# hackmad/pbrt-v3-rs

Measured on AMD Instinct MI355X. Metric: Mrays/s, higher is better.
Workload: dtype f32

## Files before the change

### pbrt-v3-rs_amd/csrc/api.hip

```cpp
#include "host_math.h"
#include "scene_host.h"
#include "traverse.h"
#include "texture.h"
#include <algorithm>
#include <cstdio>
#include <cstdlib>
#include <mutex>

static std::string g_last_error;
static std::mutex g_err_mu;

namespace phost {

int set_err(PbrtHipScene* s, int code, const std::string& msg) {
    if (s) s->err = msg;
    else { std::lock_guard<std::mutex> g(g_err_mu); g_last_error = msg; }
    return code;
}
int hip_fail(PbrtHipScene* s, hipError_t e, const char* what) {
    std::string m = std::string(what) + ": " + hipGetErrorString(e);
    (void)hipGetLastError();
    return set_err(s, e == hipErrorOutOfMemory ? PBRT_HIP_ERR_OOM : PBRT_HIP_ERR_DEVICE, m);
}
int ensure_buf(PbrtHipScene* s, DevBuf& b, size_t bytes) {
// ... 1351 lines not shown
            std::string e;
            const phost::ForestSpec spec = layout.spec(isc);
            const int brc = split_method == 1 ? phost::build_hlbvh_device(in, max_prims_in_node, s->stream, s->bvh, e, &spec, &trees)
                                              : phost::build_sah_device(in, max_prims_in_node, s->stream, s->bvh, e, &s->tree_dev_nodes, &s->tree_dev_tris, &spec, &trees);
            if (brc == -1) return set_err(s, PBRT_HIP_ERR_DEVICE, "build_accel_device: " + e);
            if (brc != 0) return fail(brc);
            if (s->tree_dev_tris) s->tree_dev_n_tris = layout.items.size();
        } else {
            const int brc = phost::build_forest_host(in, isc, layout, split_method, max_prims_in_node, s->bvh, trees);
            if (brc != 0) return fail(brc);
        }
        for (size_t k = 0; k < s->instances.size(); k++) {
            const PbrtHipScene::InstanceHost& ih = s->instances[k];
            const phost::ForestTreeOut& b = trees[layout.inst_tree[k]];
            InstRec r{};
            std::memcpy(r.w2i, ih.w2i, 64); std::memcpy(r.i2w, ih.i2w, 64);
            for (int a = 0; a < 3; a++) { r.lo[a] = b.lo[a]; r.hi[a] = b.hi[a]; }
            r.root_ref = b.root_ref; r.flags = b.n_items == 1 ? PH_INST_SINGLE : 0u;
            bool ident = true;
            for (int a = 0; a < 16; a++) if (ih.i2w[a] != ((a % 5 == 0) ? 1.0f : 0.0f)) ident = false;
            if (ident) r.flags |= PH_INST_IDENTITY;
            s->inst_recs.push_back(r);
        }
    }
    s->world_radius = 1.0f; s->world_center[0] = s->world_center[1] = s->world_center[2] = 0.0f;
    if (s->bvh.root_ref != PH_INVALID_REF) {
        const float* lo = s->bvh.root_lo; const float* hi = s->bvh.root_hi;
        float c[3];
        for (int k = 0; k < 3; k++) c[k] = (1.0f - 0.5f) * lo[k] + 0.5f * hi[k];
        bool inside = (c[0] >= lo[0] && c[0] <= hi[0]) && (c[1] >= lo[1] && c[1] <= hi[1]) && (c[2] >= lo[2] && c[2] <= hi[2]);
        float dx = c[0] - hi[0], dy = c[1] - hi[1], dz = c[2] - hi[2];
        s->world_radius = inside ? std::sqrt(dx * dx + dy * dy + dz * dz) : 0.0f;
        for (int k = 0; k < 3; k++) s->world_center[k] = c[k];
    }
    s->built = true; s->uploaded = false;
    return PBRT_HIP_OK;
    });
}

int pbrt_hip_build_accel_device(PbrtHipScene* s, int split_method, int max_prims_in_node) {
    return ph_guard(s, "pbrt_hip_build_accel_device", [&]() -> int {
    if (!s) return PBRT_HIP_ERR_INVALID_ARG;
    if (split_method != 0 && split_method != 1) return set_err(s, PBRT_HIP_ERR_UNSUPPORTED, "build_accel_device: the device builders make the SAH (0) and the HLBVH (1) tree; EqualCounts is built on the host");
    s->build_on_device = true;
    const int rc = pbrt_hip_build_accel(s, split_method, max_prims_in_node);
    s->build_on_device = false;
    return rc;
    });
}

int pbrt_hip_world_bound(const PbrtHipScene* s, float out[6]) {
    return ph_guard(const_cast<PbrtHipScene*>(s), "pbrt_hip_world_bound", [&]() -> int {
    if (!s || !out) return PBRT_HIP_ERR_INVALID_ARG;
    if (!s->built) return PBRT_HIP_ERR_STATE;
    for (int k = 0; k < 3; k++) { out[k] = s->bvh.root_lo[k]; out[3 + k] = s->bvh.root_hi[k]; }
    return PBRT_HIP_OK;
    });
}

int pbrt_hip_accel_stats(const PbrtHipScene* s, uint64_t out[8]) {
    return ph_guard(const_cast<PbrtHipScene*>(s), "pbrt_hip_accel_stats", [&]() -> int {
    if (!s || !out) return PBRT_HIP_ERR_INVALID_ARG;
    if (!s->built) return PBRT_HIP_ERR_STATE;
    out[0] = s->tree_dev_tris ? s->bvh.interior_nodes : s->bvh.nodes.size(); out[1] = s->tree_dev_tris ? s->tree_dev_n_tris : s->bvh.tris.size();
    out[2] = out[0] * sizeof(Node64); out[3] = out[1] * sizeof(TriRec);
    out[4] = s->bvh.leaf_nodes; out[5] = (uint64_t)s->bvh.max_depth; out[6] = s->bvh.max_leaf_prims;
    out[7] = (uint64_t)(s->bvh.build_seconds * 1e6);
    return PBRT_HIP_OK;
    });
}

int pbrt_hip_accel_copy(PbrtHipScene* s, void* out_nodes, uint64_t node_capacity, void* out_leaf_records, uint64_t record_capacity) {
    return ph_guard(s, "pbrt_hip_accel_copy", [&]() -> int {
    if (!s) return PBRT_HIP_ERR_INVALID_ARG;
    if (!s->built) return set_err(s, PBRT_HIP_ERR_STATE, "accel_copy: build_accel first");
    const size_t nn = s->tree_dev_tris ? s->bvh.interior_nodes : s->bvh.nodes.size(), nt = s->tree_dev_tris ? s->tree_dev_n_tris : s->bvh.tris.size();
    if (node_capacity < nn || record_capacity < nt) return set_err(s, PBRT_HIP_ERR_INVALID_ARG, "accel_copy: buffers too small (pbrt_hip_accel_stats gives the sizes)");
    if (s->tree_dev_tris) {
        PH_CHECK(s, hipSetDevice(s->device));
        if (nn && out_nodes) PH_CHECK(s, hipMemcpy(out_nodes, s->tree_dev_nodes, nn * sizeof(Node64), hipMemcpyDeviceToHost));
        if (nt && out_leaf_records) PH_CHECK(s, hipMemcpy(out_leaf_records, s->tree_dev_tris, nt * sizeof(TriRec), hipMemcpyDeviceToHost));
        if (!s->inst_recs.empty()) {
            if (out_nodes) { Node64* nd = static_cast<Node64*>(out_nodes); for (size_t i = 0; i < nn; i++) { if ((nd[i].c0 & PH_LEAF_BIT) && nd[i].c0 < PH_NEED_POP) nd[i].c0 &= ~PH_LEAF_INST_HINT; if ((nd[i].c1 & PH_LEAF_BIT) && nd[i].c1 < PH_NEED_POP) nd[i].c1 &= ~PH_LEAF_INST_HINT; } }
            if (out_leaf_records) { TriRec* tr = static_cast<TriRec*>(out_leaf_records); for (size_t i = 0; i < nt; i++) { tr[i].flags &= ~PH_TRI_NEXT_INST; if (tr[i].flags & PH_TRI_INSTANCE) { const uint32_t prim = tr[i].prim, fl = tr[i].flags; std::memset(&tr[i], 0, sizeof(TriRec)); tr[i].prim = prim; tr[i].flags = fl; } } }
        }
    } else {
        if (nn && out_nodes) std::memcpy(out_nodes, s->bvh.nodes.data(), nn * sizeof(Node64));
        if (nt && out_leaf_records) std::memcpy(out_leaf_records, s->bvh.tris.data(), nt * sizeof(TriRec));
    }
    return PBRT_HIP_OK;
    });
}

static int check_error_flag(PbrtHipScene* s) {
    uint32_t flag = 0;
    PH_CHECK(s, hipMemcpy(&flag, s->d_error.p, 4, hipMemcpyDeviceToHost));
    if (flag) {
        (void)hipMemset(s->d_error.p, 0, 4);
        return set_err(s, PBRT_HIP_ERR_DEVICE, "traversal stack exceeded 64 entries (the reference panics here, bvh/mod.rs:185)");
    }
    return PBRT_HIP_OK;
}

static int batch_common(PbrtHipScene* s, bool anyhit, const void* rays, void* out, uint64_t n, bool device_ptrs, float* kernel_ms) {
    if (!s) return PBRT_HIP_ERR_INVALID_ARG;
    if (n && (!rays || !out)) return set_err(s, PBRT_HIP_ERR_INVALID_ARG, "batch: null buffer");
    if (!s->built) return set_err(s, PBRT_HIP_ERR_STATE, "batch: call pbrt_hip_build_accel first");
    if (n > 0xFFFF0000ull) return set_err(s, PBRT_HIP_ERR_INVALID_ARG, "batch: at most 2^32-65536 rays per call");
    PH_CHECK(s, hipSetDevice(s->device));
    int rc;
    if ((rc = upload_scene(s))) return rc;
    if (n == 0) return PBRT_HIP_OK;
    const size_t out_bytes = anyhit ? (size_t)n : (size_t)n * sizeof(PbrtHipHit);
    const void* d_rays = rays; void* d_out = out;
    if (!device_ptrs) {
        if ((rc = ensure_buf(s, s->d_rays_tmp, (size_t)n * sizeof(PbrtHipRay)))) return rc;
        if ((rc = ensure_buf(s, s->d_out_tmp, out_bytes))) return rc;
        PH_CHECK(s, hipMemcpyAsync(s->d_rays_tmp.p, rays, (size_t)n * sizeof(PbrtHipRay), hipMemcpyHostToDevice, s->stream));
        d_rays = s->d_rays_tmp.p; d_out = s->d_out_tmp.p;
    }
    if ((rc = launch_traverse(s, anyhit, d_rays, d_out, (uint32_t)n, kernel_ms))) return rc;
    if (!device_ptrs) PH_CHECK(s, hipMemcpyAsync(out, d_out, out_bytes, hipMemcpyDeviceToHost, s->stream));
    PH_CHECK(s, hipStreamSynchronize(s->stream));
    return check_error_flag(s);
}

int pbrt_hip_intersect_batch(PbrtHipScene* s, const PbrtHipRay* rays, PbrtHipHit* hits, uint64_t n) { return ph_guard(s, "pbrt_hip_intersect_batch", [&]() -> int { return batch_common(s, false, rays, hits, n, false, nullptr); }); }
int pbrt_hip_occluded_batch(PbrtHipScene* s, const PbrtHipRay* rays, uint8_t* out, uint64_t n) { return ph_guard(s, "pbrt_hip_occluded_batch", [&]() -> int { return batch_common(s, true, rays, out, n, false, nullptr); }); }
int pbrt_hip_intersect_batch_device(PbrtHipScene* s, const void* d_rays, void* d_hits, uint64_t n, float* ms) { return ph_guard(s, "pbrt_hip_intersect_batch_device", [&]() -> int { return batch_common(s, false, d_rays, d_hits, n, true, ms); }); }
int pbrt_hip_occluded_batch_device(PbrtHipScene* s, const void* d_rays, void* d_occ, uint64_t n, float* ms) { return ph_guard(s, "pbrt_hip_occluded_batch_device", [&]() -> int { return batch_common(s, true, d_rays, d_occ, n, true, ms); }); }

int pbrt_hip_set_traversal_counting(PbrtHipScene* s, int on) {
    return ph_guard(s, "pbrt_hip_set_traversal_counting", [&]() -> int {
    if (!s) return PBRT_HIP_ERR_INVALID_ARG;
    PH_CHECK(s, hipSetDevice(s->device));
    int rc;
    if ((rc = ensure_traversal_workspace(s))) return rc;
    PH_CHECK(s, hipMemset(s->d_counts.p, 0, 64 + 36 * 8));
    s->count_traversal = on != 0;
    return PBRT_HIP_OK;
    });
}
int pbrt_hip_get_traversal_counts(PbrtHipScene* s, uint64_t out[8]) {
    return ph_guard(s, "pbrt_hip_get_traversal_counts", [&]() -> int {
    if (!s || !out) return PBRT_HIP_ERR_INVALID_ARG;
    if (!s->d_counts.p) { for (int i = 0; i < 8; i++) out[i] = 0; return PBRT_HIP_OK; }
    PH_CHECK(s, hipSetDevice(s->device));
    PH_CHECK(s, hipStreamSynchronize(s->stream));
    PH_CHECK(s, hipMemcpy(out, s->d_counts.p, 64, hipMemcpyDeviceToHost));
#if PH_PHASE_CLOCK
    {
        unsigned long long ph[36];
        PH_CHECK(s, hipMemcpy(ph, (const char*)s->d_counts.p + 64, sizeof ph, hipMemcpyDeviceToHost));
        static const char* names[10] = {"refill", "node_steps", "instance_entry", "triangle_test", "alpha_test", "instance_exit", "retire", "whole_loop", "stack_pops", "leaf_step_whole"};
        for (int k = 0; k < 10; k++)
            std::fprintf(stderr, "PHASE_CLOCK %-15s cycles %14llu (%5.1f %% of the loop)  executions %12llu  mean active lanes %5.1f\n", names[k], ph[k], ph[7] ? 100.0 * (double)ph[k] / (double)ph[7] : 0.0,
                         ph[12 + k], ph[12 + k] ? (double)ph[24 + k] / (double)ph[12 + k] : 0.0);
    }
    PH_CHECK(s, hipMemset(s->d_counts.p, 0, 64 + 36 * 8));
#else
    PH_CHECK(s, hipMemset(s->d_counts.p, 0, 64 + 36 * 8));
#endif
    return PBRT_HIP_OK;
    });
}

int pbrt_hip_film_to_rgb(const PbrtHipScene* s, const float* xyz, const float* weight, float* out_rgb) {
    return ph_guard(const_cast<PbrtHipScene*>(s), "pbrt_hip_film_to_rgb", [&]() -> int {
    if (!s || !xyz || !weight || !out_rgb) return PBRT_HIP_ERR_INVALID_ARG;
    if (!s->have_film) return PBRT_HIP_ERR_STATE;
    const FilmRec& f = s->film;
    const int w = f.crop[2] - f.crop[0], h = f.crop[3] - f.crop[1];
    const size_t n = (size_t)std::max(w, 0) * (size_t)std::max(h, 0);
    auto to_rgb = [](const float* x, float* r) {
        r[0] = 3.240479f * x[0] - 1.537150f * x[1] - 0.498535f * x[2];
        r[1] = -0.969256f * x[0] + 1.875991f * x[1] + 0.041556f * x[2];
        r[2] = 0.055648f * x[0] - 0.204043f * x[1] + 1.057311f * x[2];
    };
    const float zero[3] = {0, 0, 0};
    float splat_rgb[3];
    to_rgb(zero, splat_rgb);
    for (size_t i = 0; i < n; i++) {
        float rgb[3];
        to_rgb(xyz + 3 * i, rgb);
        for (int c = 0; c < 3; c++) {
            float v = rgb[c];
            if (weight[i] != 0.0f) { float inv = 1.0f / weight[i]; float q = v * inv; v = 0.0f > q ? 0.0f : q; }
            v += 1.0f * splat_rgb[0];
            v *= f.scale;
            out_rgb[3 * i + c] = v;
        }
    }
    return PBRT_HIP_OK;
    });
}

}
```

### pbrt-v3-rs_amd/csrc/traverse.h

```cpp
#pragma once
#include "dmath.h"
#include "scene_types.h"
#include "quadric.h"

constexpr int PH_TRAV_BLOCK = 256;
constexpr int PH_MAX_STACK = 64;
constexpr int PH_BATCH = 64;

namespace ph {

struct alignas(16) RayIn { float ox, oy, oz, t_max, dx, dy, dz, time; };
struct alignas(16) HitOut { float t; uint32_t prim; float b0, b1, b2; uint32_t pad[3]; };

typedef float ph_v4f __attribute__((ext_vector_type(4)));
static __device__ __forceinline__ float4 ph_stream_load(const float4* p) { const ph_v4f v = __builtin_nontemporal_load(reinterpret_cast<const ph_v4f*>(p)); return make_float4(v.x, v.y, v.z, v.w); }
static __device__ __forceinline__ uint32_t ph_stream_load(const uint32_t* p) { return __builtin_nontemporal_load(p); }
static __device__ __forceinline__ void ph_stream_store(float4 v, float4* p) { const ph_v4f w = {v.x, v.y, v.z, v.w}; __builtin_nontemporal_store(w, reinterpret_cast<ph_v4f*>(p)); }
struct TravParams {
    const RayIn* rays;
    void* out;
    uint32_t n;
    const uint32_t* n_ptr;
    uint32_t* counter;
    uint2* spill;
    uint32_t total_threads;
    uint32_t* error_flag;
    uint32_t batch;
    unsigned long long* counts;
    const RayIn* rays2; uint8_t* out2; const uint32_t* n2_ptr;
    const uint32_t* order;
    uint32_t* heads; uint32_t n_heads, head_chunk;
    unsigned long long* phase;
};

struct RayState {
    float ox, oy, oz, t_max;
    float ix, iy, iz;
    uint32_t sgn;
    float sx, sy, sz;
    PH_DEV bool nx() const { return (sgn & 1u) != 0u; }
    PH_DEV bool ny() const { return (sgn & 2u) != 0u; }
    PH_DEV bool nz() const { return (sgn & 4u) != 0u; }
    PH_DEV int kz() const { return (int)((sgn >> 3) & 3u); }
    PH_DEV int kx() const { const int k = kz() + 1; return k == 3 ? 0 : k; }
    PH_DEV int ky() const { const int k = kx() + 1; return k == 3 ? 0 : k; }
};

PH_DEV void ray_setup(RayState& r, const RayIn& in) {
    r.ox = in.ox; r.oy = in.oy; r.oz = in.oz; r.t_max = in.t_max;
    r.ix = 1.0f / in.dx; r.iy = 1.0f / in.dy; r.iz = 1.0f / in.dz;
    f3 d = mk3(in.dx, in.dy, in.dz);
    const int kz = max_dimension(vabs(d));
    r.sgn = (r.ix < 0.0f ? 1u : 0u) | (r.iy < 0.0f ? 2u : 0u) | (r.iz < 0.0f ? 4u : 0u) | ((uint32_t)kz << 3);
    f3 dp = permute(d, r.kx(), r.ky(), kz);
    r.sx = -dp.x / dp.z; r.sy = -dp.y / dp.z; r.sz = 1.0f / dp.z;
}

PH_DEV RayIn xf_ray(const float* c, const RayState& r, f3 rd, float time) {
    const float x = r.ox, y = r.oy, z = r.oz;
    const float ox = (c[0] * x + c[1] * y) + (c[2] * z + c[3]);
    const float oy = (c[4] * x + c[5] * y) + (c[6] * z + c[7]);
    const float oz = (c[8] * x + c[9] * y) + (c[10] * z + c[11]);
    const float ow = (c[12] * x + c[13] * y) + (c[14] * z + c[15]);
    const float xs = pabs(c[0] * x) + pabs(c[1] * y) + pabs(c[2] * z) + pabs(c[3]);
    const float ys = pabs(c[4] * x) + pabs(c[5] * y) + pabs(c[6] * z) + pabs(c[7]);
    const float zs = pabs(c[8] * x) + pabs(c[9] * y) + pabs(c[10] * z) + pabs(c[11]);
    const f3 o_err = kGamma3 * mk3(xs, ys, zs);
    f3 o = (ow == 1.0f) ? mk3(ox, oy, oz) : mk3(ox, oy, oz) / ow;
    const f3 d = mk3(c[0] * rd.x + c[1] * rd.y + c[2] * rd.z, c[4] * rd.x + c[5] * rd.y + c[6] * rd.z, c[8] * rd.x + c[9] * rd.y + c[10] * rd.z);
    const float l2 = length_squared(d);
    float t_max = r.t_max;
    if (l2 > 0.0f) {
        const float dt = ph_div(dot(vabs(d), o_err), l2);
        o = o + d * dt;
        t_max -= dt;
    }
    RayIn out; out.ox = o.x; out.oy = o.y; out.oz = o.z; out.t_max = t_max; out.dx = d.x; out.dy = d.y; out.dz = d.z; out.time = time;
    return out;
}

PH_DEV float vmax3(float a, float b, float c) {
#if defined(__HIP_DEVICE_COMPILE__)
    float r; asm("v_max3_f32 %0, %1, %2, %3" : "=v"(r) : "v"(a), "v"(b), "v"(c)); return r;
#else
    return a > b ? (a > c ? a : c) : (b > c ? b : c);
#endif
}
PH_DEV float vmin3(float a, float b, float c) {
#if defined(__HIP_DEVICE_COMPILE__)
    float r; asm("v_min3_f32 %0, %1, %2, %3" : "=v"(r) : "v"(a), "v"(b), "v"(c)); return r;
#else
    return a < b ? (a < c ? a : c) : (b < c ? b : c);
#endif
}

PH_DEV bool box_test(const RayState& r, float xn, float xf, float yn, float yf, float zn, float zf, float& t_min_out) {
    float t_x_min = (xn - r.ox) * r.ix;
    float t_x_max = (xf - r.ox) * r.ix;
    const float t_y_min = (yn - r.oy) * r.iy;
    float t_y_max = (yf - r.oy) * r.iy;
    t_x_max *= kBoxScale;
    t_y_max *= kBoxScale;
    const float t_z_min = (zn - r.oz) * r.iz;
    const float t_z_max = (zf - r.oz) * r.iz;
    const float t_min = vmax3(t_x_min, t_y_min, t_z_min);
    const float t_max = vmin3(t_x_max, t_y_max, t_z_max);
    t_min_out = t_min;
    return (t_min <= t_max) & (t_max > 0.0f) & ((t_x_min == t_x_min) & (t_x_max == t_x_max));
}

typedef float ph_v2f __attribute__((ext_vector_type(2)));
typedef unsigned long long ph_mask;
PH_DEV ph_mask lanes(bool c) {
#if defined(__HIP_DEVICE_COMPILE__)
    return __ballot(c);
#else
    return c ? 1ull : 0ull;
#endif
}
PH_DEV bool lane_of(ph_mask m) {
#if defined(__HIP_DEVICE_COMPILE__)
    return __builtin_amdgcn_inverse_ballot_w64(m);
#else
    return (m & 1ull) != 0ull;
#endif
}
template <int SEL> PH_DEV ph_v2f pk_sub_bcast(ph_v2f a, ph_v2f p) {
#if defined(__HIP_DEVICE_COMPILE__)
    ph_v2f d;
    if (SEL == 0) asm("v_pk_add_f32 %0, %1, %2 op_sel_hi:[1,0] neg_lo:[0,1] neg_hi:[0,1]" : "=v"(d) : "v"(a), "v"(p));
    else asm("v_pk_add_f32 %0, %1, %2 op_sel:[0,1] op_sel_hi:[1,1] neg_lo:[0,1] neg_hi:[0,1]" : "=v"(d) : "v"(a), "v"(p));
    return d;
#else
    const float o = SEL ? p.y : p.x; return (ph_v2f){a.x - o, a.y - o};
#endif
}
template <int SEL> PH_DEV ph_v2f pk_mul_bcast(ph_v2f a, ph_v2f p) {
#if defined(__HIP_DEVICE_COMPILE__)
    ph_v2f d;
    if (SEL == 0) asm("v_pk_mul_f32 %0, %1, %2 op_sel_hi:[1,0]" : "=v"(d) : "v"(a), "v"(p));
    else asm("v_pk_mul_f32 %0, %1, %2 op_sel:[0,1] op_sel_hi:[1,1]" : "=v"(d) : "v"(a), "v"(p));
    return d;
#else
    const float o = SEL ? p.y : p.x; return (ph_v2f){a.x * o, a.y * o};
#endif
}
PH_DEV void node_boxes(const RayState& r, float4 q0, float4 q1, float4 q2, ph_mask& m0, float& t0, ph_mask& m1, float& t1) {
    const ph_v2f pxy = {r.ox, r.oy}, pzi = {r.oz, r.ix}, pii = {r.iy, r.iz};
    const ph_v2f ax = pk_mul_bcast<1>(pk_sub_bcast<0>((ph_v2f){q0.x, q0.y}, pxy), pzi), ay = pk_mul_bcast<0>(pk_sub_bcast<1>((ph_v2f){q0.z, q0.w}, pxy), pii),
                 az = pk_mul_bcast<1>(pk_sub_bcast<0>((ph_v2f){q1.x, q1.y}, pzi), pii);
    const ph_v2f bx = pk_mul_bcast<1>(pk_sub_bcast<0>((ph_v2f){q1.z, q1.w}, pxy), pzi), by = pk_mul_bcast<0>(pk_sub_bcast<1>((ph_v2f){q2.x, q2.y}, pxy), pii),
                 bz = pk_mul_bcast<1>(pk_sub_bcast<0>((ph_v2f){q2.z, q2.w}, pzi), pii);
    const bool nx = r.nx(), ny = r.ny(), nz = r.nz();
    const ph_v2f scale = {kBoxScale, kBoxScale};
    const ph_v2f a_far = (ph_v2f){nx ? ax.x : ax.y, ny ? ay.x : ay.y} * scale;
    const ph_v2f b_far = (ph_v2f){nx ? bx.x : bx.y, ny ? by.x : by.y} * scale;
    t0 = vmax3(nx ? ax.y : ax.x, ny ? ay.y : ay.x, nz ? az.y : az.x);
    const float a_max = vmin3(a_far.x, a_far.y, nz ? az.x : az.y);
    t1 = vmax3(nx ? bx.y : bx.x, ny ? by.y : by.x, nz ? bz.y : bz.x);
    const float b_max = vmin3(b_far.x, b_far.y, nz ? bz.x : bz.y);
    m0 = lanes(t0 <= a_max) & lanes(a_max > 0.0f) & lanes(!__builtin_isunordered(ax.x, ax.y)) & lanes(t0 < r.t_max);
    m1 = lanes(t1 <= b_max) & lanes(b_max > 0.0f) & lanes(!__builtin_isunordered(bx.x, bx.y)) & lanes(t1 < r.t_max);
}
PH_DEV bool tri_test(const RayState& r, f3 p0, f3 p1, f3 p2, float& t_out, float& b0_out, float& b1_out, float& b2_out) {
    f3 o = mk3(r.ox, r.oy, r.oz);
    const int kx = r.kx(), ky = r.ky(), kz = r.kz();
    f3 p0t = permute(p0 - o, kx, ky, kz);
    f3 p1t = permute(p1 - o, kx, ky, kz);
    f3 p2t = permute(p2 - o, kx, ky, kz);
    p0t.x += r.sx * p0t.z; p0t.y += r.sy * p0t.z;
    p1t.x += r.sx * p1t.z; p1t.y += r.sy * p1t.z;
    p2t.x += r.sx * p2t.z; p2t.y += r.sy * p2t.z;
    float e0 = p1t.x * p2t.y - p1t.y * p2t.x;
    float e1 = p2t.x * p0t.y - p2t.y * p0t.x;
    float e2 = p0t.x * p1t.y - p0t.y * p1t.x;
    if (e0 == 0.0f || e1 == 0.0f || e2 == 0.0f) {
        double a = (double)p2t.x * (double)p1t.y, b = (double)p2t.y * (double)p1t.x;
        e0 = (float)(b - a);
        a = (double)p0t.x * (double)p2t.y; b = (double)p0t.y * (double)p2t.x;
        e1 = (float)(b - a);
        a = (double)p1t.x * (double)p0t.y; b = (double)p1t.y * (double)p0t.x;
        e2 = (float)(b - a);
    }
    if ((e0 < 0.0f || e1 < 0.0f || e2 < 0.0f) && (e0 > 0.0f || e1 > 0.0f || e2 > 0.0f)) return false;
    float det = e0 + e1 + e2;
    if (det == 0.0f) return false;
    p0t.z *= r.sz; p1t.z *= r.sz; p2t.z *= r.sz;
    float t_scaled = e0 * p0t.z + e1 * p1t.z + e2 * p2t.z;
    if (det < 0.0f && (t_scaled >= 0.0f || t_scaled < r.t_max * det)) return false;
    else if (det > 0.0f && (t_scaled <= 0.0f || t_scaled > r.t_max * det)) return false;
    float inv_det = 1.0f / det;
    float b0 = e0 * inv_det, b1 = e1 * inv_det, b2 = e2 * inv_det, t = t_scaled * inv_det;
    float max_z_t = max_component(vabs(mk3(p0t.z, p1t.z, p2t.z)));
    float delta_z = kGamma3 * max_z_t;
    float max_x_t = max_component(vabs(mk3(p0t.x, p1t.x, p2t.x)));
    float max_y_t = max_component(vabs(mk3(p0t.y, p1t.y, p2t.y)));
    float delta_x = kGamma5 * (max_x_t + max_z_t);
    float delta_y = kGamma5 * (max_y_t + max_z_t);
    float delta_e = 2.0f * (kGamma2 * max_x_t * max_y_t + delta_y * max_x_t + delta_x * max_y_t);
    float max_e = max_component(vabs(mk3(e0, e1, e2)));
    float delta_t = 3.0f * (kGamma3 * max_e * max_z_t + delta_e * max_z_t + delta_z * max_e) * fabsf(inv_det);
    if (t <= delta_t) return false;
    t_out = t; b0_out = b0; b1_out = b1; b2_out = b2;
    return true;
}

PH_DEV void tri_bary(const RayState& r, f3 p0, f3 p1, f3 p2, float& b0_out, float& b1_out, float& b2_out) {
    f3 o = mk3(r.ox, r.oy, r.oz);
    const int kx = r.kx(), ky = r.ky(), kz = r.kz();
    f3 p0t = permute(p0 - o, kx, ky, kz);
    f3 p1t = permute(p1 - o, kx, ky, kz);
    f3 p2t = permute(p2 - o, kx, ky, kz);
    p0t.x += r.sx * p0t.z; p0t.y += r.sy * p0t.z;
    p1t.x += r.sx * p1t.z; p1t.y += r.sy * p1t.z;
    p2t.x += r.sx * p2t.z; p2t.y += r.sy * p2t.z;
    float e0 = p1t.x * p2t.y - p1t.y * p2t.x;
    float e1 = p2t.x * p0t.y - p2t.y * p0t.x;
    float e2 = p0t.x * p1t.y - p0t.y * p1t.x;
    if (e0 == 0.0f || e1 == 0.0f || e2 == 0.0f) {
        double a = (double)p2t.x * (double)p1t.y, b = (double)p2t.y * (double)p1t.x;
        e0 = (float)(b - a);
        a = (double)p0t.x * (double)p2t.y; b = (double)p0t.y * (double)p2t.x;
        e1 = (float)(b - a);
        a = (double)p1t.x * (double)p0t.y; b = (double)p1t.y * (double)p0t.x;
        e2 = (float)(b - a);
    }
    const float det = e0 + e1 + e2;
    const float inv_det = 1.0f / det;
    b0_out = e0 * inv_det; b1_out = e1 * inv_det; b2_out = e2 * inv_det;
}

#ifndef PH_PHASE_CLOCK
#define PH_PHASE_CLOCK 0
#endif
#include "phase_clock.h"
static __device__ __noinline__ bool alpha_accept(const DeviceScene* dsc, uint32_t tri_index, float b0, float b1, float b2, uint32_t any_hit);
static __device__ __forceinline__ void alpha_general_prepare();
static __device__ __forceinline__ bool alpha_accept_lean(const DeviceScene& sc, uint32_t prim, uint32_t mesh, float b0, float b1, float b2, bool any_hit);
enum TravMode : int { TRAV_CLOSEST = 0, TRAV_ANY = 1, TRAV_MIXED = 2 };

struct ShapeDefaults {
    static constexpr bool count = false, inst = false, quadric = false;
    static constexpr int leaf_min = 20, refill_min = 12;
    static constexpr int lds_depth = 12;
    static constexpr int node_steps = 1;
    static constexpr int alpha = 0, alpha_min = 0, wpe = 0;
};
struct ShapeFlat : ShapeDefaults { static constexpr int leaf_min = 16, refill_min = 32, node_steps = 6, wpe = 6; };
struct ShapeInst : ShapeDefaults { static constexpr bool inst = true; static constexpr int leaf_min = 24, lds_depth = 11, node_steps = 5, wpe = 5; };
struct ShapeFlatAlphaLean : ShapeDefaults { static constexpr int leaf_min = 24, node_steps = 5, alpha = 1, alpha_min = 12; };
struct ShapeInstAlphaLean : ShapeDefaults { static constexpr bool inst = true; static constexpr int leaf_min = 16, lds_depth = 11, node_steps = 5, alpha = 1, alpha_min = 12, wpe = 5; };
template <bool INST> struct ShapeAlphaGeneral : ShapeDefaults { static constexpr bool inst = INST; static constexpr int node_steps = 3, alpha = 2, alpha_min = 12; };
struct ShapeQuadric : ShapeFlat { static constexpr bool quadric = true; static constexpr int wpe = 0; };
struct ShapeQuadricAlphaLean : ShapeQuadric { static constexpr int alpha = 1, alpha_min = 12; };
struct ShapeQuadricAlphaGeneral : ShapeQuadric { static constexpr int alpha = 2, alpha_min = 12; };
template <bool INST, int ALPHA, bool QUADRIC = false> struct ShapeCount : ShapeDefaults { static constexpr bool count = true, inst = INST, quadric = QUADRIC; static constexpr int alpha = ALPHA; };

template <class... S> struct ShapeTable {
    static constexpr int find(bool inst, int alpha, bool quadric, bool count) { int i = 0, at = -1; ((at = (S::inst == inst && S::alpha == alpha && S::quadric == quadric && S::count == count) ? i : at, i++), ...); return at; }
    static constexpr int spill_lds_depth(bool inst) { int d = PH_MAX_STACK; ((d = (S::inst == inst && S::lds_depth < d) ? S::lds_depth : d), ...); return d; }
};
using TravShapes = ShapeTable<ShapeFlat, ShapeInst, ShapeFlatAlphaLean, ShapeInstAlphaLean, ShapeAlphaGeneral<false>, ShapeAlphaGeneral<true>, ShapeQuadric,
                              ShapeCount<false, 0>, ShapeCount<true, 0>, ShapeCount<false, 1>, ShapeCount<true, 1>, ShapeCount<false, 2>, ShapeCount<true, 2>, ShapeCount<false, 0, true>,
                              ShapeQuadricAlphaLean, ShapeQuadricAlphaGeneral, ShapeCount<false, 1, true>, ShapeCount<false, 2, true>>;
constexpr int pick_shape(bool inst, int alpha, bool quadric, bool count) { return quadric ? TravShapes::find(false, alpha, true, count) : TravShapes::find(inst, alpha, false, count); }
constexpr bool every_scene_has_a_shape() {
    for (int k = 0; k < 24; k++) if (pick_shape(k & 1, (k >> 1) % 3, k >= 12, k % 12 >= 6) < 0) return false;
    return true;
}
static_assert(every_scene_has_a_shape(), "a combination of scene features has no row in TravShapes");
constexpr int trav_stack_cap(bool inst) { return inst ? 2 * PH_MAX_STACK : PH_MAX_STACK; }

template <class Shape, int MODE>
__global__ __launch_bounds__(PH_TRAV_BLOCK) __attribute__((amdgpu_waves_per_eu(Shape::wpe ? Shape::wpe : 1, Shape::wpe ? Shape::wpe : 8))) void traverse_kernel(DeviceScene sc, TravParams p) {
    constexpr bool ANYHIT = MODE == TRAV_ANY, MIXED = MODE == TRAV_MIXED, COUNT = Shape::count, INST = Shape::inst, QUADRIC = Shape::quadric;
    constexpr int LEAF_MIN = Shape::leaf_min, REFILL_MIN = Shape::refill_min, LDS_DEPTH = Shape::lds_depth, NODE_STEPS = Shape::node_steps, ALPHA = Shape::alpha, ALPHA_MIN = Shape::alpha_min;
    static_assert(MODE == TRAV_CLOSEST || MODE == TRAV_ANY || MODE == TRAV_MIXED, "no such mode");
    static_assert(LDS_DEPTH >= TravShapes::spill_lds_depth(INST), "the spill region starts at the shallowest LDS stack of the table's rows: a shape outside the table would write past it");
    static_assert(ALPHA_MIN == 0 || ALPHA != 0, "the alpha phase needs an alpha test");
    static_assert(!QUADRIC || !INST, "build_accel refuses quadrics together with instances: no such kernel");
    __shared__ uint2 lds_stack[LDS_DEPTH][PH_TRAV_BLOCK];
    __shared__ float inst_save[INST ? 9 : 1][INST ? PH_TRAV_BLOCK : 1];
    const uint32_t tid = threadIdx.x;
#if PH_PHASE_CLOCK && defined(__HIP_DEVICE_COMPILE__)
    __shared__ unsigned long long phc_lds[36];
    if (tid < 36) phc_lds[tid] = 0ull;
    __syncthreads();
#endif
    PHC_BEGIN(7);
    if (ALPHA == 2) alpha_general_prepare();
    const uint32_t lane = tid & 63u;
    const uint32_t gtid = blockIdx.x * PH_TRAV_BLOCK + tid;
    const uint64_t lane_lt = (lane == 0) ? 0ull : (~0ull >> (64 - lane));
    const uint32_t n_first = p.n_ptr ? *p.n_ptr : p.n;
    const uint32_t n_rays = MIXED ? n_first + *p.n2_ptr : n_first;
    bool ah = ANYHIT;

    bool has_ray = false;
    uint32_t batch_next = 0, batch_end = 0;
    bool exhausted = false;
    uint32_t head_cur = p.n_heads > 1u ? blockIdx.x % p.n_heads : 0u, heads_dry = 0u;
    uint32_t ray_index = 0;
    RayState r;
    uint32_t cur = PH_INVALID_REF;
    int sp = 0;
    constexpr bool LEAN = !INST;
    uint32_t hit_prim = 0xFFFFFFFFu, hit_tri = LEAN ? 0xFFFFFFFFu : 0u, hit_cls = 0u;
    float hb0 = 0.0f, hb1 = 0.0f, hb2 = 0.0f;
    bool occluded = false;
    uint32_t c_nodes[2] = {0, 0}, c_tris[2] = {0, 0}, c_rays[2] = {0, 0}, c_visits = 0, c_culled = 0;
    float wdx = 0.0f, wdy = 0.0f, wdz = 0.0f;
    uint32_t in_inst = 0;
    int inst_sp = 0;
    float world_tmax = 0.0f;
    uint32_t cont_ref = PH_INVALID_REF;
    bool inst_hit = false;
    uint32_t hit_inst = 0;
    bool alpha_wait = false;

    auto push = [&](uint32_t ref, float tmin) {
        uint2 e = make_uint2(ref, __float_as_uint(tmin));
        if (sp < LDS_DEPTH) lds_stack[sp][tid] = e;
        else if (sp < trav_stack_cap(INST)) p.spill[(size_t)(sp - LDS_DEPTH) * p.total_threads + gtid] = e;
        else { *p.error_flag = 1u; return; }
        sp++;
    };
    auto owe_pop = [&]() -> uint32_t {
        const int floor_sp = (INST && in_inst) ? inst_sp : 0;
        return sp > floor_sp ? PH_NEED_POP : PH_INVALID_REF;
    };
    auto pop_once = [&]() {
        const int floor_sp = (INST && in_inst) ? inst_sp : 0;
        if (sp > floor_sp) {
            sp--;
            uint2 e;
            if (sp < LDS_DEPTH) { e = lds_stack[sp][tid]; asm volatile("; stack entry from LDS" : "+v"(e.x), "+v"(e.y)); }
            else { e = p.spill[(size_t)(sp - LDS_DEPTH) * p.total_threads + gtid]; asm volatile("; stack entry from the spill region" : "+v"(e.x), "+v"(e.y)); }
            if (COUNT && ah) c_visits++;
            if (COUNT && !(__uint_as_float(e.y) < r.t_max)) c_culled++;
            cur = (__uint_as_float(e.y) < r.t_max) ? e.x : PH_NEED_POP;
        } else cur = PH_INVALID_REF;
    };

    auto retire = [&]() {
            PHC_BEGIN(6);
            if (MIXED && ah) p.out2[ray_index - n_first] = occluded ? 1 : 0;
            else if (!MIXED && ANYHIT) reinterpret_cast<uint8_t*>(p.out)[ray_index] = occluded ? 1 : 0;
            else {
                float4* hp = reinterpret_cast<float4*>(reinterpret_cast<HitOut*>(p.out) + ray_index);
                if (LEAN) {
                    if (hit_tri != 0xFFFFFFFFu) {
                        const float4* tp = reinterpret_cast<const float4*>(sc.tris + hit_tri);
                        const float4 a = tp[0], b = tp[1], c = tp[2];
                        if (QUADRIC && (__float_as_uint(b.w) & PH_TRI_QUADRIC)) hb0 = hb1 = hb2 = 0.0f;
                        else
                        tri_bary(r, mk3(a.x, a.y, a.z), mk3(b.x, b.y, b.z), mk3(c.x, c.y, c.z), hb0, hb1, hb2);
                        hit_prim = __float_as_uint(a.w); hit_cls = (__float_as_uint(b.w) >> PH_TRI_CLASS_SHIFT) & PH_TRI_KEY_MASK;
                    } else { hit_prim = 0xFFFFFFFFu; hit_tri = 0u; hit_cls = 0u; hb0 = hb1 = hb2 = 0.0f; }
                }
                ph_stream_store(make_float4(r.t_max, __uint_as_float(hit_prim), hb0, hb1), hp);
                ph_stream_store(make_float4(hb2, __uint_as_float(hit_tri), __uint_as_float(INST ? hit_inst : 0u), __uint_as_float(hit_cls)), hp + 1);
            }
            has_ray = false;
            if (COUNT) c_rays[(MIXED && ah) ? 1 : 0]++;
            PHC_END(6);
    };

    for (;;) {
        {
            PHC_BEGIN(0);
            const bool finished = has_ray && cur == PH_INVALID_REF && !(INST && in_inst);
            const uint64_t idle = __ballot(!has_ray || finished);
            const uint32_t n_idle = (uint32_t)__popcll(idle);
            if (n_idle >= (uint32_t)REFILL_MIN || n_idle == 64u || (n_idle && __ballot(has_ray && !finished) == 0ull)) {
                if (finished) retire();
                if (batch_next == batch_end && !exhausted) {
                    if (p.n_heads > 1u) {
                        uint32_t b = 0;
                        if (lane == 0) b = atomicAdd(p.heads + 16u * head_cur, p.batch);
                        b = __shfl(b, 0);
                        const uint32_t chunk = b / p.head_chunk;
                        const uint64_t q = ((uint64_t)chunk * p.n_heads + head_cur) * p.head_chunk + (b - chunk * p.head_chunk);
                        if (q < (uint64_t)n_rays) { batch_next = (uint32_t)q; batch_end = ((uint32_t)q + p.batch < n_rays) ? (uint32_t)q + p.batch : n_rays; }
                        else {
                            heads_dry++; head_cur = head_cur + 1u == p.n_heads ? 0u : head_cur + 1u;
                            if (heads_dry >= p.n_heads) exhausted = true;
                        }
                    } else {
                        uint32_t b = 0;
                        if (lane == 0) b = atomicAdd(p.counter, p.batch);
                        b = __shfl(b, 0);
                        if (b >= n_rays) exhausted = true;
                        else { batch_next = b; batch_end = (b + p.batch < n_rays) ? b + p.batch : n_rays; }
                    }
                }
                const uint32_t avail = batch_end - batch_next;
                if (avail) {
                    const uint32_t rank = (uint32_t)__popcll(idle & lane_lt);
                    if (!has_ray && rank < avail) {
                        ray_index = p.order ? ph_stream_load(p.order + batch_next + rank) : batch_next + rank;
                        if (MIXED) ah = ray_index >= n_first;
                        const float4* rp = reinterpret_cast<const float4*>((MIXED && ah) ? p.rays2 + (ray_index - n_first) : p.rays + ray_index);
                        const float4 a = ph_stream_load(rp), b = ph_stream_load(rp + 1);
                        RayIn in; in.ox = a.x; in.oy = a.y; in.oz = a.z; in.t_max = a.w; in.dx = b.x; in.dy = b.y; in.dz = b.z; in.time = b.w;
                        ray_setup(r, in);
                        has_ray = true; sp = 0; occluded = false; alpha_wait = false;
                        if (LEAN) hit_tri = 0xFFFFFFFFu; else { hit_prim = 0xFFFFFFFFu; hit_tri = 0u; hb0 = hb1 = hb2 = 0.0f; }
                        if (INST) { in_inst = 0; hit_inst = 0; wdx = in.dx; wdy = in.dy; wdz = in.dz; }
                        cur = PH_INVALID_REF;
                        if (COUNT && ah) c_visits++;
                        if (sc.root_ref != PH_INVALID_REF) {
                            float tmin;
                            const bool h = box_test(r, r.nx() ? sc.root_hi[0] : sc.root_lo[0], r.nx() ? sc.root_lo[0] : sc.root_hi[0],
                                                    r.ny() ? sc.root_hi[1] : sc.root_lo[1], r.ny() ? sc.root_lo[1] : sc.root_hi[1],
                                                    r.nz() ? sc.root_hi[2] : sc.root_lo[2], r.nz() ? sc.root_lo[2] : sc.root_hi[2], tmin);
                            if (h && tmin < r.t_max) cur = sc.root_ref;
                        }
                    }
                    batch_next += (n_idle < avail) ? n_idle : avail;
                }
                PHC_END(0);
            }
        }
        if (__ballot(has_ray) == 0ull) {
            if (exhausted && batch_next == batch_end) break;
            continue;
        }

#pragma unroll
        for (int step = 0; step < NODE_STEPS; step++) {
        if (has_ray && cur == PH_NEED_POP) { PHC_BEGIN(8); pop_once(); PHC_END(8); }
        if (has_ray && !(cur & PH_LEAF_BIT)) {
            PHC_BEGIN(1);
            const float4* np = reinterpret_cast<const float4*>(sc.nodes + cur);
            const float4 q0 = np[0], q1 = np[1], q2 = np[2];
            const uint4 q3 = reinterpret_cast<const uint4*>(np)[3];
            if (COUNT) c_nodes[(MIXED && ah) ? 1 : 0]++;
            float t0, t1;
            ph_mask m0, m1;
            node_boxes(r, q0, q1, q2, m0, t0, m1, t1);
#if defined(__HIP_DEVICE_COMPILE__)
            const ph_mask m_neg = lanes(__builtin_amdgcn_ubfe(r.sgn, q3.z, 1u) != 0u);
#else
            const ph_mask m_neg = lanes(((r.sgn >> q3.z) & 1u) != 0u);
#endif
            const bool neg_axis = lane_of(m_neg);
            const uint32_t near_ref = neg_axis ? q3.y : q3.x, far_ref = neg_axis ? q3.x : q3.y;
            const bool near_hit = lane_of((m_neg & m1) | (~m_neg & m0)), far_hit = lane_of((m_neg & m0) | (~m_neg & m1));
            const float far_t = neg_axis ? t0 : t1;
            if (COUNT && ah) {
                if (near_hit) { c_visits++; if (!far_hit) push(far_ref, __builtin_nanf("")); }
                else c_visits += 2;
            }
            if (near_hit) { cur = near_ref; if (far_hit) push(far_ref, far_t); }
            else if (far_hit) cur = far_ref;
            else cur = owe_pop();
            PHC_END(1);
        }
        }

        {
            const bool waiting = ALPHA && ALPHA_MIN > 0 && has_ray && alpha_wait;
            const bool at_leaf = has_ray && cur < PH_NEED_POP && (cur & PH_LEAF_BIT) && !waiting;
            const uint64_t lm = __ballot(at_leaf), am = (ALPHA && ALPHA_MIN > 0) ? __ballot(waiting) : 0ull;
            if ((lm | am) != 0ull) {
                const uint64_t nm = __ballot(has_ray && (cur == PH_NEED_POP || !(cur & PH_LEAF_BIT)));
                const bool fire_leaf = lm != 0ull && ((uint32_t)__popcll(lm) >= (uint32_t)LEAF_MIN || nm == 0ull || exhausted);
                const bool fire_alpha = am != 0ull && ((uint32_t)__popcll(am) >= (uint32_t)(ALPHA_MIN > 0 ? ALPHA_MIN : 1) || nm == 0ull || exhausted);
                if (fire_leaf || fire_alpha) {
                    if ((at_leaf && fire_leaf) || (waiting && fire_alpha)) {
                        PHC_BEGIN(9);
                        const uint32_t ti = INST ? (cur & ~(PH_LEAF_BIT | PH_LEAF_INST_HINT)) : (cur & ~PH_LEAF_BIT);
                        const float4* tp = reinterpret_cast<const float4*>(sc.tris + ti);
                        const float4 a = tp[0], b = tp[1], c = tp[2];
                        const bool hinted = INST && (cur & PH_LEAF_INST_HINT) != 0u;
                        float4 e0 = make_float4(0.0f, 0.0f, 0.0f, 0.0f), e1 = e0, e2 = e0;
                        if (INST && hinted) { const float4* ep = reinterpret_cast<const float4*>(sc.inst_extra) + 3u * (size_t)ti; e0 = ep[0]; e1 = ep[1]; e2 = ep[2]; }
                        const uint32_t flags = __float_as_uint(b.w);
                        bool last = (flags & PH_TRI_LAST) != 0;
                        const uint32_t next_ref = INST ? (((cur & ~PH_LEAF_INST_HINT) + 1u) | ((flags & PH_TRI_NEXT_INST) ? PH_LEAF_INST_HINT : 0u)) : cur + 1u;
                        float t, b0, b1, b2;
                        if (INST && (flags & PH_TRI_INSTANCE)) {
                            PHC_BEGIN(2);
                            if (!hinted) { const float4* ep = reinterpret_cast<const float4*>(sc.inst_extra) + 3u * (size_t)ti; e0 = ep[0]; e1 = ep[1]; e2 = ep[2]; }
                            const uint32_t iflags = __float_as_uint(c.y), iroot = __float_as_uint(c.x);
                            float w2i[16] = {e0.x, e0.y, e0.z, e0.w, e1.x, e1.y, e1.z, e1.w, e2.x, e2.y, e2.z, e2.w, 0.0f, 0.0f, 0.0f, 1.0f};
                            if (iflags & PH_INST_GENERAL) { const InstRec& I = sc.instances[__float_as_uint(a.w)]; for (int k = 12; k < 16; k++) w2i[k] = I.w2i[k]; }
                            world_tmax = r.t_max; cont_ref = last ? PH_INVALID_REF : next_ref;
                            in_inst = (__float_as_uint(a.w) + 1u) | ((r.sgn >> 3) << 30); inst_sp = sp; inst_hit = false;
                            inst_save[0][tid] = r.ox; inst_save[1][tid] = r.oy; inst_save[2][tid] = r.oz;
                            inst_save[3][tid] = r.ix; inst_save[4][tid] = r.iy; inst_save[5][tid] = r.iz; inst_save[6][tid] = r.sx; inst_save[7][tid] = r.sy; inst_save[8][tid] = r.sz;
                            const RayIn in = xf_ray(w2i, r, mk3(wdx, wdy, wdz), 0.0f);
                            ray_setup(r, in);
                            cur = PH_INVALID_REF;
                            if (iflags & PH_INST_SINGLE) cur = iroot;
                            else {
                                float tmin;
                                const bool h = box_test(r, r.nx() ? b.x : a.x, r.nx() ? a.x : b.x, r.ny() ? b.y : a.y, r.ny() ? a.y : b.y,
                                                        r.nz() ? b.z : a.z, r.nz() ? a.z : b.z, tmin);
                                if (h && tmin < r.t_max) cur = iroot;
                            }
                            PHC_END(2);
                        } else {
                        PHC_BEGIN(3);
                        if (COUNT) c_tris[(MIXED && ah) ? 1 : 0]++;
                        const bool second_meeting = ALPHA && ALPHA_MIN > 0 && alpha_wait;
                        alpha_wait = false;
                        auto quadric_leaf = [&]() -> bool {
                            const float4 rdq = reinterpret_cast<const float4*>((MIXED && ah) ? p.rays2 + (ray_index - n_first) : p.rays + ray_index)[1];
                            t = quadric_test(sc.self, __float_as_uint(a.x), r.ox, r.oy, r.oz, r.t_max, rdq.x, rdq.y, rdq.z);
                            b0 = b1 = b2 = 0.0f;
                            return t > 0.0f;
                        };
                        if ((QUADRIC && (flags & PH_TRI_QUADRIC)) ? quadric_leaf() : tri_test(r, mk3(a.x, a.y, a.z), mk3(b.x, b.y, b.z), mk3(c.x, c.y, c.z), t, b0, b1, b2)) {
                            const uint32_t reject = ah ? (PH_TRI_BOGUS | PH_TRI_ALPHA0 | PH_TRI_SALPHA0) : (PH_TRI_BOGUS | PH_TRI_ALPHA0);
                            bool accept = !(flags & reject);
                            if (ALPHA && accept && (flags & PH_TRI_ALPHATEX)) {
                                if (ALPHA_MIN > 0 && !second_meeting) { alpha_wait = true; accept = false; }
                                else {
                                PHC_BEGIN(4);
                                accept = ALPHA == 1 ? alpha_accept_lean(sc, __float_as_uint(a.w), __float_as_uint(c.w), b0, b1, b2, ah) : alpha_accept(sc.self, ti, b0, b1, b2, ah ? 1u : 0u);
                                PHC_END(4);
                                }
                            }
                            if (accept) {
                                if (ah) occluded = true;
                                else {
                                    r.t_max = t; hit_tri = ti;
                                    if (!LEAN) { hit_prim = __float_as_uint(a.w); hb0 = b0; hb1 = b1; hb2 = b2; hit_cls = (flags >> PH_TRI_CLASS_SHIFT) & PH_TRI_KEY_MASK; }
                                    if (INST) { hit_inst = in_inst & 0x3FFFFFFFu; inst_hit = true; }
                                }
                            }
                        }
                        if (ALPHA && ALPHA_MIN > 0 && alpha_wait) { }
                        else if (ah && occluded) cur = PH_INVALID_REF;
                        else if (last) cur = owe_pop();
                        else cur = next_ref;
                        PHC_END(3);
                        }
                        PHC_END(9);
                    }
                }
            }
        }

        if (INST && has_ray && in_inst && cur == PH_INVALID_REF) {
            PHC_BEGIN(5);
            if (!(ah && occluded)) {
                const float t_new = inst_hit ? r.t_max : world_tmax;
                r.ox = inst_save[0][tid]; r.oy = inst_save[1][tid]; r.oz = inst_save[2][tid];
                r.ix = inst_save[3][tid]; r.iy = inst_save[4][tid]; r.iz = inst_save[5][tid]; r.sx = inst_save[6][tid]; r.sy = inst_save[7][tid]; r.sz = inst_save[8][tid];
                r.sgn = (r.ix < 0.0f ? 1u : 0u) | (r.iy < 0.0f ? 2u : 0u) | (r.iz < 0.0f ? 4u : 0u) | ((in_inst >> 30) << 3);
                r.t_max = t_new;
                in_inst = 0;
                cur = (cont_ref != PH_INVALID_REF) ? cont_ref : owe_pop();
            } else in_inst = 0;
            PHC_END(5);
        }

    }
    PHC_END(7);
#if PH_PHASE_CLOCK && defined(__HIP_DEVICE_COMPILE__)
    __syncthreads();
    if (tid < 36 && p.phase) atomicAdd(p.phase + tid, phc_lds[tid]);
#endif
    if (COUNT) {
        const int k0 = (!MIXED && ANYHIT) ? 3 : 0;
        atomicAdd(p.counts + k0 + 0, (unsigned long long)c_nodes[0]);
        atomicAdd(p.counts + k0 + 1, (unsigned long long)c_tris[0]);
        atomicAdd(p.counts + k0 + 2, (unsigned long long)c_rays[0]);
        if (MIXED) {
            atomicAdd(p.counts + 3, (unsigned long long)c_nodes[1]);
            atomicAdd(p.counts + 4, (unsigned long long)c_tris[1]);
            atomicAdd(p.counts + 5, (unsigned long long)c_rays[1]);
        }
        atomicAdd(p.counts + 6, (unsigned long long)c_visits);
        atomicAdd(p.counts + 7, (unsigned long long)c_culled);
    }
// ... 4 lines not shown
```

Baseline: 2326.

## Stage ray batches ahead in registers for flat traversal kernel refill

Adds a staged refill state machine for the flat kernel. Across loop iterations it claims the next batch with an atomic, loads the order indices, and prefetches ray data into per-lane registers. Idle lanes then pull rays from those registers by shuffle instead of waiting on global loads at refill time. The goal is to hide the atomic and memory latency of refill behind traversal work, at the cost of extra registers and some per-iteration state-machine overhead.

```diff
diff --git a/pbrt-v3-rs_amd/csrc/api.hip b/pbrt-v3-rs_amd/csrc/api.hip
--- a/pbrt-v3-rs_amd/csrc/api.hip
+++ b/pbrt-v3-rs_amd/csrc/api.hip
@@ -1527,8 +1527,8 @@
     {
         unsigned long long ph[36];
         PH_CHECK(s, hipMemcpy(ph, (const char*)s->d_counts.p + 64, sizeof ph, hipMemcpyDeviceToHost));
-        static const char* names[10] = {"refill", "node_steps", "instance_entry", "triangle_test", "alpha_test", "instance_exit", "retire", "whole_loop", "stack_pops", "leaf_step_whole"};
-        for (int k = 0; k < 10; k++)
+        static const char* names[11] = {"refill", "node_steps", "instance_entry", "triangle_test", "alpha_test", "instance_exit", "retire", "whole_loop", "stack_pops", "leaf_step_whole", "stage_ahead"};
+        for (int k = 0; k < 11; k++)
             std::fprintf(stderr, "PHASE_CLOCK %-15s cycles %14llu (%5.1f %% of the loop)  executions %12llu  mean active lanes %5.1f\n", names[k], ph[k], ph[7] ? 100.0 * (double)ph[k] / (double)ph[7] : 0.0,
                          ph[12 + k], ph[12 + k] ? (double)ph[24 + k] / (double)ph[12 + k] : 0.0);
     }
diff --git a/pbrt-v3-rs_amd/csrc/refill_plan.h b/pbrt-v3-rs_amd/csrc/refill_plan.h
--- /dev/null
+++ b/pbrt-v3-rs_amd/csrc/refill_plan.h
@@ -0,0 +1,77 @@
+#pragma once
+#include <cstdint>
+
+#if defined(__HIPCC__)
+#define PH_RP_FN __host__ __device__ __forceinline__
+#else
+#define PH_RP_FN inline
+#endif
+
+namespace ph {
+
+enum RefillStage : uint32_t { RP_CLAIM = 0, RP_CLAIMED = 1, RP_INDEXED = 2, RP_LOADING = 3, RP_READY = 4 };
+enum RefillDo : uint32_t { RP_DO_NOTHING = 0, RP_DO_CLAIM = 1, RP_DO_INDEX = 2, RP_DO_LOAD = 3 };
+
+struct RefillQueue { uint32_t n_rays, batch, n_heads, head_chunk; };
+struct RefillPlan {
+    uint32_t stage;
+    uint32_t q0, q_n;
+    uint32_t staged_next;
+    uint32_t head_cur, heads_dry;
+    bool drained;
+};
+
+PH_RP_FN RefillPlan refill_plan_start(const RefillQueue& q, uint32_t block) {
+    RefillPlan p;
+    p.stage = RP_CLAIM; p.q0 = 0u; p.q_n = 0u; p.staged_next = 0u;
+    p.head_cur = q.n_heads > 1u ? block % q.n_heads : 0u; p.heads_dry = 0u;
+    p.drained = false;
+    return p;
+}
+
+PH_RP_FN uint32_t refill_claim_slot(const RefillPlan& p) { return p.head_cur; }
+
+PH_RP_FN uint32_t refill_step(const RefillQueue& q, RefillPlan& p, uint32_t claimed) {
+    if (p.stage == RP_CLAIM) {
+        if (p.drained) return RP_DO_NOTHING;
+        p.stage = RP_CLAIMED;
+        return RP_DO_CLAIM;
+    }
+    if (p.stage == RP_CLAIMED) {
+        uint64_t pos = claimed;
+        if (q.n_heads > 1u) {
+            const uint32_t chunk = claimed / q.head_chunk;
+            pos = ((uint64_t)chunk * q.n_heads + p.head_cur) * q.head_chunk + (claimed - chunk * q.head_chunk);
+        }
+        if (pos < (uint64_t)q.n_rays) {
+            const uint32_t left = q.n_rays - (uint32_t)pos;
+            p.q0 = (uint32_t)pos; p.q_n = left < q.batch ? left : q.batch; p.staged_next = 0u;
+            p.stage = RP_INDEXED;
+            return RP_DO_INDEX;
+        }
+        p.stage = RP_CLAIM;
+        if (q.n_heads > 1u) {
+            p.heads_dry++; p.head_cur = p.head_cur + 1u == q.n_heads ? 0u : p.head_cur + 1u;
+            if (p.heads_dry >= q.n_heads) p.drained = true;
+        } else p.drained = true;
+        return RP_DO_NOTHING;
+    }
+    if (p.stage == RP_INDEXED) { p.stage = RP_LOADING; return RP_DO_LOAD; }
+    if (p.stage == RP_LOADING) p.stage = RP_READY;
+    return RP_DO_NOTHING;
+}
+
+PH_RP_FN uint32_t refill_lane_position(const RefillPlan& p, uint32_t lane) { return p.q0 + (lane < p.q_n ? lane : p.q_n - 1u); }
+
+PH_RP_FN uint32_t refill_available(const RefillPlan& p) { return p.stage == RP_READY ? p.q_n - p.staged_next : 0u; }
+PH_RP_FN uint32_t refill_staged_next(const RefillPlan& p) { return p.staged_next; }
+PH_RP_FN uint32_t refill_take(RefillPlan& p, uint32_t n_idle) {
+    const uint32_t avail = refill_available(p), n = n_idle < avail ? n_idle : avail;
+    p.staged_next += n;
+    if (avail && p.staged_next == p.q_n) p.stage = RP_CLAIM;
+    return n;
+}
+
+PH_RP_FN bool refill_drained(const RefillPlan& p) { return p.drained && p.stage == RP_CLAIM; }
+
+}
diff --git a/pbrt-v3-rs_amd/csrc/traverse.h b/pbrt-v3-rs_amd/csrc/traverse.h
--- a/pbrt-v3-rs_amd/csrc/traverse.h
+++ b/pbrt-v3-rs_amd/csrc/traverse.h
@@ -2,6 +2,7 @@
 #include "dmath.h"
 #include "scene_types.h"
 #include "quadric.h"
+#include "refill_plan.h"
 
 constexpr int PH_TRAV_BLOCK = 256;
 constexpr int PH_MAX_STACK = 64;
@@ -123,6 +124,13 @@
     return __builtin_amdgcn_inverse_ballot_w64(m);
 #else
     return (m & 1ull) != 0ull;
+#endif
+}
+PH_DEV uint32_t first_lane(uint32_t v) {
+#if defined(__HIP_DEVICE_COMPILE__)
+    return (uint32_t)__builtin_amdgcn_readfirstlane((int)v);
+#else
+    return v;
 #endif
 }
 template <int SEL> PH_DEV ph_v2f pk_sub_bcast(ph_v2f a, ph_v2f p) {
@@ -245,13 +253,14 @@
     static constexpr int lds_depth = 12;
     static constexpr int node_steps = 1;
     static constexpr int alpha = 0, alpha_min = 0, wpe = 0;
+    static constexpr bool stage_ahead = false;
 };
-struct ShapeFlat : ShapeDefaults { static constexpr int leaf_min = 16, refill_min = 32, node_steps = 6, wpe = 6; };
+struct ShapeFlat : ShapeDefaults { static constexpr int leaf_min = 16, refill_min = 32, node_steps = 6, wpe = 6; static constexpr bool stage_ahead = true; };
 struct ShapeInst : ShapeDefaults { static constexpr bool inst = true; static constexpr int leaf_min = 24, lds_depth = 11, node_steps = 5, wpe = 5; };
 struct ShapeFlatAlphaLean : ShapeDefaults { static constexpr int leaf_min = 24, node_steps = 5, alpha = 1, alpha_min = 12; };
 struct ShapeInstAlphaLean : ShapeDefaults { static constexpr bool inst = true; static constexpr int leaf_min = 16, lds_depth = 11, node_steps = 5, alpha = 1, alpha_min = 12, wpe = 5; };
 template <bool INST> struct ShapeAlphaGeneral : ShapeDefaults { static constexpr bool inst = INST; static constexpr int node_steps = 3, alpha = 2, alpha_min = 12; };
-struct ShapeQuadric : ShapeFlat { static constexpr bool quadric = true; static constexpr int wpe = 0; };
+struct ShapeQuadric : ShapeFlat { static constexpr bool quadric = true, stage_ahead = false; static constexpr int wpe = 0; };
 struct ShapeQuadricAlphaLean : ShapeQuadric { static constexpr int alpha = 1, alpha_min = 12; };
 struct ShapeQuadricAlphaGeneral : ShapeQuadric { static constexpr int alpha = 2, alpha_min = 12; };
 template <bool INST, int ALPHA, bool QUADRIC = false> struct ShapeCount : ShapeDefaults { static constexpr bool count = true, inst = INST, quadric = QUADRIC; static constexpr int alpha = ALPHA; };
@@ -279,6 +288,9 @@
     static_assert(LDS_DEPTH >= TravShapes::spill_lds_depth(INST), "the spill region starts at the shallowest LDS stack of the table's rows: a shape outside the table would write past it");
     static_assert(ALPHA_MIN == 0 || ALPHA != 0, "the alpha phase needs an alpha test");
     static_assert(!QUADRIC || !INST, "build_accel refuses quadrics together with instances: no such kernel");
+    constexpr bool STAGE_AHEAD = Shape::stage_ahead;
+    static_assert(!STAGE_AHEAD || (!COUNT && !INST && !QUADRIC && ALPHA == 0), "the staged refill is written for the flat kernel only");
+    static_assert(PH_BATCH == 64, "a staged batch is one ray per lane of the wave");
     __shared__ uint2 lds_stack[LDS_DEPTH][PH_TRAV_BLOCK];
     __shared__ float inst_save[INST ? 9 : 1][INST ? PH_TRAV_BLOCK : 1];
     const uint32_t tid = threadIdx.x;
@@ -301,6 +313,10 @@
     bool exhausted = false;
     uint32_t head_cur = p.n_heads > 1u ? blockIdx.x % p.n_heads : 0u, heads_dry = 0u;
     uint32_t ray_index = 0;
+    const RefillQueue rq = {n_rays, (uint32_t)PH_BATCH, p.n_heads, p.head_chunk};
+    RefillPlan rp = refill_plan_start(rq, blockIdx.x);
+    uint32_t st_claim = 0u, st_idx = 0u;
+    ph_v4f st_a = {0.0f, 0.0f, 0.0f, 0.0f}, st_b = st_a;
     RayState r;
     uint32_t cur = PH_INVALID_REF;
     int sp = 0;
@@ -367,7 +383,63 @@
     };
 
     for (;;) {
-        {
+        if constexpr (STAGE_AHEAD) {
+            const bool finished = has_ray && cur == PH_INVALID_REF;
+            const uint64_t idle = __ballot(!has_ray || finished);
+            const uint32_t n_idle = (uint32_t)__popcll(idle);
+            if (n_idle >= (uint32_t)REFILL_MIN || n_idle == 64u || (n_idle && __ballot(has_ray && !finished) == 0ull)) {
+                PHC_BEGIN(0);
+                const uint32_t avail = refill_available(rp);
+                uint32_t idx = 0u;
+                RayIn in = {};
+                const uint32_t rank = (uint32_t)__popcll(idle & lane_lt);
+                if (avail) {
+                    const int src = (int)(refill_staged_next(rp) + (rank < avail ? rank : 0u));
+                    idx = (uint32_t)__shfl((int)st_idx, src);
+                    in.ox = __shfl(st_a.x, src); in.oy = __shfl(st_a.y, src); in.oz = __shfl(st_a.z, src); in.t_max = __shfl(st_a.w, src);
+                    in.dx = __shfl(st_b.x, src); in.dy = __shfl(st_b.y, src); in.dz = __shfl(st_b.z, src); in.time = __shfl(st_b.w, src);
+                }
+                if (finished) retire();
+                if (avail) {
+                    if (!has_ray && rank < avail) {
+                        ray_index = idx;
+                        if (MIXED) ah = ray_index >= n_first;
+                        ray_setup(r, in);
+                        has_ray = true; sp = 0; occluded = false;
+                        hit_tri = 0xFFFFFFFFu;
+                        cur = PH_INVALID_REF;
+                        if (sc.root_ref != PH_INVALID_REF) {
+                            float tmin;
+                            const bool h = box_test(r, r.nx() ? sc.root_hi[0] : sc.root_lo[0], r.nx() ? sc.root_lo[0] : sc.root_hi[0],
+                                                    r.ny() ? sc.root_hi[1] : sc.root_lo[1], r.ny() ? sc.root_lo[1] : sc.root_hi[1],
+                                                    r.nz() ? sc.root_hi[2] : sc.root_lo[2], r.nz() ? sc.root_lo[2] : sc.root_hi[2], tmin);
+                            if (h && tmin < r.t_max) cur = sc.root_ref;
+                        }
+                    }
+                    refill_take(rp, n_idle);
+                }
+                PHC_END(0);
+            }
+            PHC_BEGIN(10);
+            const uint32_t claimed = rp.stage == RP_CLAIMED ? first_lane(st_claim) : 0u;
+            const uint32_t what = first_lane(refill_step(rq, rp, claimed));
+            if (what == RP_DO_CLAIM) {
+                uint32_t zero = 0u;
+                asm volatile("; the claim's address as a per-lane value" : "+v"(zero));
+                uint32_t* const head = (p.n_heads > 1u ? p.heads + 16u * refill_claim_slot(rp) : p.counter) + zero;
+                if (lane == 0) st_claim = atomicAdd(head, (uint32_t)PH_BATCH);
+            }
+            if (what == RP_DO_INDEX) {
+                const uint32_t pos = refill_lane_position(rp, lane);
+                st_idx = p.order ? ph_stream_load(p.order + pos) : pos;
+            }
+            if (what == RP_DO_LOAD) {
+                const ph_v4f* sp_ray = reinterpret_cast<const ph_v4f*>((MIXED && st_idx >= n_first) ? p.rays2 + (st_idx - n_first) : p.rays + st_idx);
+                st_a = __builtin_nontemporal_load(sp_ray); st_b = __builtin_nontemporal_load(sp_ray + 1);
+            }
+            exhausted = refill_drained(rp);
+            PHC_END(10);
+        } else {
             PHC_BEGIN(0);
             const bool finished = has_ray && cur == PH_INVALID_REF && !(INST && in_inst);
             const uint64_t idle = __ballot(!has_ray || finished);
@@ -423,7 +495,7 @@
             }
         }
         if (__ballot(has_ray) == 0ull) {
-            if (exhausted && batch_next == batch_end) break;
+            if (STAGE_AHEAD ? exhausted : (exhausted && batch_next == batch_end)) break;
             continue;
         }
 
```

Measured after the change: 2335, median of 6. No clear change (+0.4%).
